# thebarnable/sparch

Measured on AMD Instinct MI355X. Metric: train-step timesteps*samples/sec (fwd+bwd+Adam), RadLIF 3x1024 SSC shape, higher is better.
Workload: dtype f32; 1 GPU; RadLIF [1024, 1024, 35] batchnorm pdrop=0.1, B=256/GPU T=250 C=700 Bernoulli(0.05) spikes (BASELINE.json configs[2]); global_batch=256, seq_len=250, parallelism=dp1, sync_bn=False, launch=eager (auto: host enqueue 2.58 ms of a 6.64 ms step during warm-up), operands=fp32 through exact bf16 splits

## Files before the change

sparch_amd/csrc/gemm_spike.hip:

```cpp
#include <cstdlib>
#include <type_traits>
#include "common.h"

namespace {

typedef unsigned u32x4 __attribute__((ext_vector_type(4)));
typedef unsigned u32x2 __attribute__((ext_vector_type(2)));
typedef short s16x4 __attribute__((ext_vector_type(4)));
typedef __bf16 bf16x8 __attribute__((ext_vector_type(8)));
typedef __attribute__((address_space(3))) s16x4 lds_s16x4;

constexpr int BK = 32;
constexpr int TAIL2 = 2;
constexpr int KC_ROW = 40;
template <int ROWS> constexpr int km_row() { return ROWS + 32; }
template <bool KM, int ROWS> constexpr int plane_elems() { return KM ? BK * km_row<ROWS>() : ROWS * KC_ROW; }

enum Epi { EPI_NONE = 0, EPI_BIAS = 1, EPI_STATS = 2 };

#ifdef SPARCH_REC_PROF
__device__ unsigned long long g_gemm_prof[8 + 8 * 2];
#define GP_DECL                                                                                  \
    unsigned long long gp_t = 0, gp_acc[5] = {0, 0, 0, 0, 0}, gp_c0, gp_r0;                      \
    asm volatile("s_memtime %0\n\ts_memrealtime %1\n\ts_waitcnt lgkmcnt(0)" : "=s"(gp_c0), "=s"(gp_r0)::"memory");
#define GP_STAMP(i)                                                                              \
    do {                                                                                         \
        unsigned long long now_;                                                                 \
        __builtin_amdgcn_sched_barrier(0);                                                       \
        asm volatile("s_memtime %0\n\ts_waitcnt lgkmcnt(0)" : "=s"(now_)::"memory");           \
        __builtin_amdgcn_sched_barrier(0);                                                       \
        if ((i) >= 0) gp_acc[(i) < 0 ? 0 : (i)] += now_ - gp_t;                                  \
        gp_t = now_;                                                                             \
    } while (0)
#define GP_FLUSH()                                                                               \
    if ((threadIdx.x & 63) == 0 && blockIdx.x == 7) {                                            \
        atomicAdd(&g_gemm_prof[8 + 2 * (threadIdx.x >> 6)], gp_acc[3]);                          \
        atomicAdd(&g_gemm_prof[9 + 2 * (threadIdx.x >> 6)], gp_acc[4]);                          \
    }                                                                                            \
    if (threadIdx.x == 0 && blockIdx.x == 7) {                                                   \
        unsigned long long c1_, r1_;                                                             \
        asm volatile("s_memtime %0\n\ts_memrealtime %1\n\ts_waitcnt lgkmcnt(0)" : "=s"(c1_), "=s"(r1_)::"memory"); \
        for (int i_ = 0; i_ < 5; ++i_) atomicAdd(&g_gemm_prof[i_], gp_acc[i_]);                  \
        atomicAdd(&g_gemm_prof[5], c1_ - gp_c0);                                                 \
        atomicAdd(&g_gemm_prof[6], r1_ - gp_r0);                                                 \
    }
#else
#define GP_DECL
#define GP_STAMP(i)
#define GP_FLUSH()
#endif

struct SArgs {
    const float* A; const float* B; float* C;
    const float* bias; float* colstat;
    int M, N, K, lda, ldb, ldc;
    int k_per_split; size_t c_split_stride;
    int a_vec, b_vec;
    float scale;
    const unsigned* gate; unsigned gate_want;
    int e_exact;
    const unsigned short* Bp; size_t bp_stride;
    const unsigned short* Ap; size_t ap_stride;
    int n_splits;
};

__device__ __forceinline__ unsigned short bf16_bits(float x) {
    return __builtin_bit_cast(unsigned short, (__bf16)x);
}
__device__ __forceinline__ void split3(float x, unsigned short& hi, unsigned short& mid, unsigned short& lo) {
    const __bf16 h = (__bf16)x;
    const float r1 = x - (float)h;
    const __bf16 m = (__bf16)r1;
    const float r2 = r1 - (float)m;
    hi = __builtin_bit_cast(unsigned short, h);
    mid = __builtin_bit_cast(unsigned short, m);
    lo = bf16_bits(r2);
}

template <bool KM, int ROWS>
__device__ __forceinline__ bool tile_is_full(int row0, int rows, int k0, int kend, int vec) {
    return vec && row0 + ROWS <= rows && k0 + BK <= kend;
}
__device__ __forceinline__ f32x4 ld16(const void* q) { return *reinterpret_cast<const f32x4*>(q); }
template <int PPR>
__device__ __forceinline__ void rm_piece(int f, int& row, int& kp) { row = f / PPR; kp = f % PPR; }
template <bool KM, int ROWS, int NT>
__device__ __forceinline__ void load_piece(f32x4& out, int p, bool fast, const float* __restrict__ P, int ld,
                                           int row0, int rows, int k0, int kend, int vec, int tid) {
    constexpr int RQ = ROWS / 4;
    const int f = tid + NT * p;
    int row, k;
    if constexpr (!KM) { int r_, kp_; rm_piece<8>(f, r_, kp_); row = row0 + r_; k = k0 + (kp_ << 2); }
    else               { k = k0 + f / RQ; row = row0 + ((f % RQ) << 2); }
    if (fast) {
        if constexpr (!KM) out = ld16(P + (size_t)row * ld + k);
        else               out = ld16(P + (size_t)k * ld + row);
        return;
    }
    f32x4 v = {0.f, 0.f, 0.f, 0.f};
    if constexpr (!KM) {
        if (row < rows) {
            const float* q = P + (size_t)row * ld + k;
            if (vec && k + 3 < kend) v = *reinterpret_cast<const f32x4*>(q);
            else {
                if (k + 0 < kend) v.x = q[0];
                if (k + 1 < kend) v.y = q[1];
                if (k + 2 < kend) v.z = q[2];
                if (k + 3 < kend) v.w = q[3];
            }
        }
    } else {
        if (k < kend) {
            const float* q = P + (size_t)k * ld + row;
            if (vec && row + 3 < rows) v = *reinterpret_cast<const f32x4*>(q);
            else {
                if (row + 0 < rows) v.x = q[0];
// ... 76 lines not shown
            const float r0 = r[2 * pr] - __uint_as_float(x0 & 0xFFFF0000u);
            const float r1 = r[2 * pr + 1] - __uint_as_float(x1 & 0xFFFF0000u);
            const unsigned y0 = __float_as_uint(r0), y1 = __float_as_uint(r1);
            const float q0 = r0 - __uint_as_float(y0 & 0xFFFF0000u);
            const float q1 = r1 - __uint_as_float(y1 & 0xFFFF0000u);
            w1[pr] = __builtin_amdgcn_perm(x1, x0, 0x07060302u);
            w2[pr] = __builtin_amdgcn_perm(y1, y0, 0x07060302u);
            w3[pr] = __builtin_amdgcn_perm(__float_as_uint(q1), __float_as_uint(q0), 0x07060302u);
        }
        *reinterpret_cast<u32x2*>(S + off) = w1;
        *reinterpret_cast<u32x2*>(S + PLANE + off) = w2;
        *reinterpret_cast<u32x2*>(S + 2 * PLANE + off) = w3;
    } else {
        unsigned short h[4], m[4], l[4];
#pragma unroll
        for (int e = 0; e < 4; ++e) split3(r[e], h[e], m[e], l[e]);
        *reinterpret_cast<u32x2*>(S + off) = u32x2{(unsigned)h[0] | ((unsigned)h[1] << 16), (unsigned)h[2] | ((unsigned)h[3] << 16)};
        *reinterpret_cast<u32x2*>(S + PLANE + off) = u32x2{(unsigned)m[0] | ((unsigned)m[1] << 16), (unsigned)m[2] | ((unsigned)m[3] << 16)};
        *reinterpret_cast<u32x2*>(S + 2 * PLANE + off) = u32x2{(unsigned)l[0] | ((unsigned)l[1] << 16), (unsigned)l[2] | ((unsigned)l[3] << 16)};
    }
}
template <bool KM, int ROWS, int NT>
__device__ __forceinline__ void store_piece_rne1(const f32x4& r, int p, unsigned short* __restrict__ S, int tid) {
    constexpr int RQ = ROWS / 4;
    typedef __bf16 bf16x2 __attribute__((ext_vector_type(2)));
    const int f = tid + NT * p;
    int off;
    if constexpr (!KM) { int r_, kp_; rm_piece<8>(f, r_, kp_); off = r_ * KC_ROW + (kp_ << 2); }
    else               off = (f / RQ) * km_row<ROWS>() + ((f % RQ) << 2);
    u32x2 w;
    w.x = __builtin_bit_cast(unsigned, bf16x2{(__bf16)r.x, (__bf16)r.y});
    w.y = __builtin_bit_cast(unsigned, bf16x2{(__bf16)r.z, (__bf16)r.w});
    *reinterpret_cast<u32x2*>(S + off) = w;
}
template <bool KM, int ROWS>
__device__ __forceinline__ u32x4 frag_read(const unsigned short* __restrict__ S, int idx_base, int lane, int ks) {
    constexpr int KM_ROW = km_row<ROWS>();
    if constexpr (!KM) {
        const int r = lane & 31, h = lane >> 5;
        return *reinterpret_cast<const u32x4*>(S + (idx_base + r) * KC_ROW + 16 * ks + 8 * h);
    } else {
        const int g = lane >> 4, i = lane & 15, q = i >> 2, p4 = i & 3;
        const int col = idx_base + 16 * (g & 1) + 4 * p4;
        const int k0 = 16 * ks + 8 * (g >> 1);
        const unsigned short* a0 = S + (k0 + q) * KM_ROW + col;
        const u32x2 lo = __builtin_bit_cast(u32x2, __builtin_amdgcn_ds_read_tr16_b64_v4i16((lds_s16x4*)(a0)));
        const u32x2 hi = __builtin_bit_cast(u32x2, __builtin_amdgcn_ds_read_tr16_b64_v4i16((lds_s16x4*)(a0 + 4 * KM_ROW)));
        return u32x4{lo.x, lo.y, hi.x, hi.y};
    }
}

__device__ __forceinline__ f32x16 mfma_bf16(u32x4 a, u32x4 b, f32x16 c) {
    return __builtin_amdgcn_mfma_f32_32x32x16_bf16(__builtin_bit_cast(bf16x8, a), __builtin_bit_cast(bf16x8, b), c, 0, 0, 0);
}

template <int MODE, bool FAST, bool BIG = false> struct Shape {
    static constexpr int WM = FAST ? (MODE == 1 ? 4 : 2) : 2;
    static constexpr int WN = FAST ? (MODE == 1 ? 2 : 4) : 2;
    static constexpr int WI = FAST ? (MODE == 0 ? 4 : (MODE == 1 ? (BIG ? 2 : 1) : (BIG ? 4 : 2))) : 2;
    static constexpr int WJ = FAST ? (MODE == 1 ? 4 : (BIG ? 2 : 1)) : 2;
    static constexpr int BM = 32 * WI * WM, BN = 32 * WJ * WN;
    static constexpr int NT = 64 * WM * WN;
    static constexpr int OCC = FAST ? 1 : (MODE == 2 ? 2 : 3);
};

template <bool A_KM, bool B_KM, int MODE, bool FAST, int NP>
constexpr bool big_tile() { return FAST && ((A_KM && B_KM && MODE != 2) || NP == 1); }

extern __shared__ __attribute__((aligned(16))) unsigned short dyn_lds[];

template <bool A_KM, bool B_KM, int MODE, bool FAST, int NP = 3>
constexpr int stage_elems() {
    using S = Shape<MODE, FAST, big_tile<A_KM, B_KM, MODE, FAST, NP>()>;
    return (MODE == 0 ? 1 : NP) * plane_elems<A_KM, S::BM>() + (MODE == 1 ? 1 : NP) * plane_elems<B_KM, S::BN>();
}

template <bool A_KM, bool B_KM, int MODE, int EPI, bool FAST, bool S16, bool BPRE = false, int NP = 3, bool APRE = false>
__global__ __launch_bounds__((Shape<MODE, FAST>::NT), (Shape<MODE, FAST>::OCC)) void gemm_spike_kernel(SArgs g) {
    static_assert(!S16 || MODE != 2, "a bf16 plane is a spike operand");
    static_assert(!BPRE || (FAST && MODE != 1), "pre-split B: pipelined kernel, B is the dense operand");
    static_assert(!APRE || (FAST && MODE != 0 && NP == 3), "pre-split A: pipelined exact kernel, A is the dense operand");
    static_assert(NP == 3 || (NP == 1 && !BPRE), "dense operands: three exact planes or one rounded plane");
    constexpr bool BIGT = big_tile<A_KM, B_KM, MODE, FAST, NP>();
    using S = Shape<MODE, FAST, BIGT>;
    constexpr bool SPIKE_A = MODE == 0;
    constexpr bool SPIKE_B = MODE == 1;
    constexpr int WI = S::WI, WJ = S::WJ, WN = S::WN, BM = S::BM, BN = S::BN, NT = S::NT;
    constexpr int A_PLANES = SPIKE_A ? 1 : NP;
    [[maybe_unused]] constexpr int B_PLANES = SPIKE_B ? 1 : NP;
    constexpr int PLANE_A = plane_elems<A_KM, BM>(), PLANE_B = plane_elems<B_KM, BN>();
    constexpr int STAGE = stage_elems<A_KM, B_KM, MODE, FAST, NP>();
    unsigned short* const lds = dyn_lds;

    if (g.gate != nullptr && *g.gate != g.gate_want) return;
    const int tid = threadIdx.x;
    const int lane = tid & 63, wave = tid >> 6;
    const int li = lane & 31, h = lane >> 5;
    const int wm = wave / WN, wn = wave % WN;
    const int tiles_n = (g.N + BN - 1) / BN;
    const int tiles_all = tiles_n * ((g.M + BM - 1) / BM);
    const int total = tiles_all * g.n_splits;
    const int xcd = blockIdx.x & 7, idx = blockIdx.x >> 3;
    const int wgs_here = (gridDim.x >> 3) + (xcd < (int)(gridDim.x & 7) ? 1 : 0);
    const int lin_end = (xcd + 1) * (total >> 3) + min(xcd + 1, total & 7);
    constexpr bool WALKS = FAST && !BIGT;
    int lin = xcd * (total >> 3) + min(xcd, total & 7) + idx;
// ... 227 lines not shown
    for (int j = 0; j < WJ; ++j) {
        csum[j] = 0.f; csq[j] = 0.f;
        const int col = n0 + (wn * WJ + j) * 32 + li;
        float bj = 0.f;
        if constexpr (EPI & EPI_BIAS) bj = (g.bias != nullptr && (FAST || col < g.N)) ? g.bias[col] : 0.f;
#pragma unroll
        for (int i = 0; i < WI; ++i) {
#pragma unroll
            for (int r = 0; r < 16; ++r) {
                const int row = m0 + (wm * WI + i) * 32 + (r & 3) + 8 * (r >> 2) + 4 * h;
                float v = acc[i][j][r] * g.scale;
                if constexpr (EPI & EPI_BIAS) v = v + bj;
                if (FAST || (row < g.M && col < g.N)) {
                    Cz[(size_t)row * g.ldc + col] = v;
                    if constexpr (EPI & EPI_STATS) { csum[j] += v; csq[j] += v * v; }
                }
            }
        }
    }
    if constexpr (EPI & EPI_STATS) {
        float* red = reinterpret_cast<float*>(lds);
#pragma unroll
        for (int j = 0; j < WJ; ++j) {
            csum[j] += __shfl_xor(csum[j], 32);
            csq[j] += __shfl_xor(csq[j], 32);
        }
        if (h == 0) {
#pragma unroll
            for (int j = 0; j < WJ; ++j) {
                const int c = (wn * WJ + j) * 32 + li;
                red[(0 * 2 + wm) * BN + c] = csum[j];
                red[(1 * 2 + wm) * BN + c] = csq[j];
            }
        }
        __syncthreads();
        if (tid < BN && n0 + tid < g.N && g.colstat != nullptr) {
            const int blocks = (g.M + 127) / 128;
            if constexpr (WI == 2) {
                g.colstat[(size_t)tile_m * g.N + n0 + tid] = red[0 * BN + tid] + red[1 * BN + tid];
                g.colstat[(size_t)(blocks + tile_m) * g.N + n0 + tid] = red[2 * BN + tid] + red[3 * BN + tid];
            } else {
                static_assert(WI == 2 || WI == 4, "colstat blocks are 128 rows");
#pragma unroll
                for (int w = 0; w < 2; ++w) {
                    const int blk = 2 * tile_m + w;
                    if (blk < blocks) {
                        g.colstat[(size_t)blk * g.N + n0 + tid] = red[(0 * 2 + w) * BN + tid];
                        g.colstat[(size_t)(blocks + blk) * g.N + n0 + tid] = red[(1 * 2 + w) * BN + tid];
                    }
                }
            }
        }
    }
    __syncthreads();
    } while (WALKS && (lin += wgs_here) < lin_end);
}

__global__ void splitk_reduce_kernel2(const float* __restrict__ ws, float* __restrict__ C, int M, int N, int ldc,
                                      int splits, int zero_diag, int accumulate, int ld_ws = 0) {
    const size_t i = (size_t)blockIdx.x * blockDim.x + threadIdx.x;
    const size_t total = (size_t)M * N;
    if (i >= total) return;
    const int m = (int)(i / N), n = (int)(i % N);
    const size_t lw = ld_ws ? (size_t)ld_ws : (size_t)N, slab = (size_t)M * lw, at = (size_t)m * lw + n;
    float s = 0.f;
    for (int z = 0; z < splits; ++z) s += ws[(size_t)z * slab + at];
    if (zero_diag && m == n) s = 0.f;
    float* c = C + (size_t)m * ldc + n;
    *c = accumulate ? (*c + s) : s;
}

int target_wgs(int occ) {
    static const int env = [] { const char* e = getenv("SPARCH_GEMM_TARGET_WGS"); return e ? atoi(e) : 0; }();
    if (env > 0) return env;
    static const int cus = [] {
        int dev = 0, n = 256;
        if (hipGetDevice(&dev) == hipSuccess) (void)hipDeviceGetAttribute(&n, hipDeviceAttributeMultiprocessorCount, dev);
        return n;
    }();
    return occ * cus;
}
template <int MODE>
int choose_splits(int M, int N, int K) {
    if (sparch_operand_bf16()) {
        using SB = Shape<MODE, true, true>;
        const int tiles_b = cdiv(M, SB::BM) * cdiv(N, SB::BN);
        int sb = target_wgs(1) / tiles_b;
        if (sb > cdiv(K, BK) / 8) sb = cdiv(K, BK) / 8;
        return sb < 1 ? 1 : sb;
    }
    using S = Shape<MODE, true, MODE != 2>;
    const int tiles = cdiv(M, S::BM) * cdiv(N, S::BN);
    const int kt = cdiv(K, BK);
    int s = target_wgs(1) / tiles;
    if (s > kt / 8) s = kt / 8;
    return s < 1 ? 1 : s;
}

template <bool A_KM, bool B_KM, int MODE, int EPI, bool S16, int NP = 3>
bool fast_ok(const SArgs& g) {
    using S = Shape<MODE, true, big_tile<A_KM, B_KM, MODE, true, NP>()>;
    constexpr int BM = S::BM, BN = S::BN;
    constexpr int QA = (S16 && MODE == 0) ? 8 : 4, QB = (S16 && MODE == 1) ? 8 : 4;
    return g.a_vec && g.b_vec && g.M >= BM && g.N >= BN && (!A_KM || g.M % QA == 0) && (!B_KM || g.N % QB == 0) &&
           (!(EPI & EPI_STATS) || g.M % BM == 0) && g.k_per_split % BK == 0 &&
           g.k_per_split >= 8 * BK;
}

template <bool A_KM, bool B_KM, int MODE, int EPI, bool FAST, bool S16, bool BPRE = false, int NP = 3, bool APRE = false>
int launch_variant(SArgs& g, int splits, hipStream_t st) {
    constexpr bool BIGT = big_tile<A_KM, B_KM, MODE, FAST, NP>();
    using S = Shape<MODE, FAST, BIGT>;
    const int work = cdiv(g.M, S::BM) * cdiv(g.N, S::BN) * splits;
    g.n_splits = splits;
    static const bool persistent = [] { const char* e = getenv("SPARCH_GEMM_PERSISTENT"); return !e || atoi(e) != 0; }();
    const int cus = target_wgs(1);
    const int wgs = (FAST && !BIGT && persistent && work > cus) ? cus : work;
    constexpr size_t lds_bytes = (size_t)(FAST ? 2 : 1) * stage_elems<A_KM, B_KM, MODE, FAST, NP>() * sizeof(unsigned short);
    auto kernel = gemm_spike_kernel<A_KM, B_KM, MODE, EPI, FAST, S16, BPRE, NP, APRE>;
    static const hipError_t attr = hipFuncSetAttribute(reinterpret_cast<const void*>(kernel),
                                                       hipFuncAttributeMaxDynamicSharedMemorySize, (int)lds_bytes);
    if (attr != hipSuccess) { sparch_note_hip_error((int)attr); return SPARCH_ELAUNCH; }
    hipLaunchKernelGGL(kernel, dim3(wgs, 1, 1), dim3(Shape<MODE, FAST>::NT), lds_bytes, st, g);
    SPARCH_CHECK_LAUNCH();
    return SPARCH_OK;
}

template <bool A_KM, bool B_KM, int MODE, int EPI, bool S16 = false>
int launch(SArgs& g, int splits, hipStream_t st) {
    if (sparch_operand_bf16()) {
        if (fast_ok<A_KM, B_KM, MODE, EPI, S16, 1>(g))
            return launch_variant<A_KM, B_KM, MODE, EPI, true, S16, false, 1>(g, splits, st);
        return launch_variant<A_KM, B_KM, MODE, EPI, false, S16, false, 1>(g, splits, st);
    }
    if (fast_ok<A_KM, B_KM, MODE, EPI, S16>(g)) return launch_variant<A_KM, B_KM, MODE, EPI, true, S16>(g, splits, st);
    return launch_variant<A_KM, B_KM, MODE, EPI, false, S16>(g, splits, st);
}
template <bool A_KM, bool B_KM, int MODE, int EPI, bool S16 = false>
int launch_wp(SArgs& g, int splits, hipStream_t st) {
    const bool planes_ok = g.Bp != nullptr && aligned16(g.Bp) && g.ldb % 8 == 0 && (g.bp_stride % 8) == 0 &&
                           g.k_per_split % BK == 0 && g.K % BK == 0 && (!B_KM || g.N % 8 == 0);
    if (planes_ok && !sparch_operand_bf16() && fast_ok<A_KM, B_KM, MODE, EPI, S16>(g))
        return launch_variant<A_KM, B_KM, MODE, EPI, true, S16, true>(g, splits, st);
    return launch<A_KM, B_KM, MODE, EPI, S16>(g, splits, st);
}

template <bool A_KM, bool B_KM, int MODE, int EPI, bool S16, bool BPRE>
int launch_ap(SArgs& g, int splits, hipStream_t st) {
    const bool a_ok = g.Ap != nullptr && aligned16(g.Ap) && g.lda % 8 == 0 && (g.ap_stride % 8) == 0 &&
// ... 29 lines not shown
}

}

extern "C" int sparch_split3(size_t n, const float* x, uint16_t* planes, void* stream) {
    SPARCH_ENTER();
    if (n == 0 || n % 8 != 0 || !x || !planes) return SPARCH_EINVAL;
    if (!aligned16(x) || !aligned16(planes)) return SPARCH_EALIGN;
    const size_t n4 = n / 4;
    hipLaunchKernelGGL(split3_kernel, dim3((unsigned)((n4 + 255) / 256)), dim3(256), 0, (hipStream_t)stream, n4,
                       reinterpret_cast<const u32x4*>(x), reinterpret_cast<u32x2*>(planes),
                       reinterpret_cast<u32x2*>(planes + n), reinterpret_cast<u32x2*>(planes + 2 * n));
    SPARCH_CHECK_LAUNCH();
    return SPARCH_OK;
}

extern "C" int sparch_gemm_spike_nt(int M, int N, int K, const float* A_spk, int lda, float scale, const float* B,
                                    int ldb, float* C, int ldc, const float* bias, float* colstat_ws,
                                    void* stream, int precision) {
    SPARCH_ENTER();
    PrecisionScope prec_scope_(precision);
    if (!prec_scope_.ok) return SPARCH_EINVAL;
    if (M <= 0 || N <= 0 || K <= 0 || !A_spk || !B || !C || lda < K || ldb < K || ldc < N) return SPARCH_EINVAL;
    SArgs g{};
    g.A = A_spk; g.B = B; g.C = C; g.bias = bias; g.colstat = colstat_ws;
    g.M = M; g.N = N; g.K = K; g.lda = lda; g.ldb = ldb; g.ldc = ldc;
    g.k_per_split = cdiv(K, BK) * BK; g.c_split_stride = 0; g.scale = scale;
    g.a_vec = aligned16(A_spk) && (lda % 4 == 0);
    g.b_vec = aligned16(B) && (ldb % 4 == 0);
    hipStream_t st = (hipStream_t)stream;
    if (colstat_ws) return launch<false, false, 0, EPI_BIAS | EPI_STATS>(g, 1, st);
    if (bias) return launch<false, false, 0, EPI_BIAS>(g, 1, st);
    return launch<false, false, 0, EPI_NONE>(g, 1, st);
}

extern "C" int sparch_gemm_spike_tn(int M, int N, int K, const float* A, int lda, const float* B, int ldb,
                                    int spike_side, float scale, float* C, int ldc, int zero_diag,
                                    int accumulate, void* ws, size_t ws_bytes, void* stream, int precision) {
    SPARCH_ENTER();
    PrecisionScope prec_scope_(precision);
    if (!prec_scope_.ok) return SPARCH_EINVAL;
    if (M <= 0 || N <= 0 || K <= 0 || !A || !B || !C || lda < M || ldb < N || ldc < N) return SPARCH_EINVAL;
    if (spike_side != 0 && spike_side != 1) return SPARCH_EINVAL;
    hipStream_t st = (hipStream_t)stream;
    const int splits = spike_side == 0 ? choose_splits<0>(M, N, K) : choose_splits<1>(M, N, K);
    const size_t need = (size_t)splits * M * N * sizeof(float);
    if (!ws || ws_bytes < need) return SPARCH_EWORKSPACE;
    SArgs g{};
    g.A = A; g.B = B; g.M = M; g.N = N; g.K = K; g.lda = lda; g.ldb = ldb; g.scale = scale;
    g.a_vec = aligned16(A) && (lda % 4 == 0);
    g.b_vec = aligned16(B) && (ldb % 4 == 0);
    g.C = (float*)ws; g.ldc = N; g.c_split_stride = (size_t)M * N;
    g.k_per_split = cdiv(cdiv(K, splits), BK) * BK;
    int rc = spike_side == 0 ? launch<true, true, 0, EPI_NONE>(g, splits, st)
                             : launch<true, true, 1, EPI_NONE>(g, splits, st);
    if (rc != SPARCH_OK) return rc;
    const size_t total = (size_t)M * N;
    hipLaunchKernelGGL(splitk_reduce_kernel2, dim3((unsigned)((total + 255) / 256)), dim3(256), 0, st,
                       (const float*)ws, C, M, N, ldc, splits, zero_diag, accumulate);
    SPARCH_CHECK_LAUNCH();
    return SPARCH_OK;
}

extern "C" int sparch_gemm_spike16_nt(int M, int N, int K, const uint16_t* A_spk16, int lda, float scale,
                                      const float* B, int ldb, float* C, int ldc, const float* bias,
                                      float* colstat_ws, void* stream, int precision) {
    SPARCH_ENTER();
    PrecisionScope prec_scope_(precision);
    if (!prec_scope_.ok) return SPARCH_EINVAL;
    if (M <= 0 || N <= 0 || K <= 0 || !A_spk16 || !B || !C || lda < K || ldb < K || ldc < N) return SPARCH_EINVAL;
    SArgs g{};
    g.A = reinterpret_cast<const float*>(A_spk16); g.B = B; g.C = C; g.bias = bias; g.colstat = colstat_ws;
    g.M = M; g.N = N; g.K = K; g.lda = lda; g.ldb = ldb; g.ldc = ldc;
    g.k_per_split = cdiv(K, BK) * BK; g.c_split_stride = 0; g.scale = scale;
    g.a_vec = aligned16(A_spk16) && (lda % 8 == 0);
    g.b_vec = aligned16(B) && (ldb % 4 == 0);
    hipStream_t st = (hipStream_t)stream;
    if (colstat_ws) return launch<false, false, 0, EPI_BIAS | EPI_STATS, true>(g, 1, st);
    if (bias) return launch<false, false, 0, EPI_BIAS, true>(g, 1, st);
    return launch<false, false, 0, EPI_NONE, true>(g, 1, st);
}

extern "C" int sparch_gemm_spike16_nt_wp(int M, int N, int K, const uint16_t* A_spk16, int lda, float scale,
                                         const float* B, const uint16_t* B_planes, int ldb, float* C, int ldc,
                                         const float* bias, float* colstat_ws, void* stream, int precision) {
    SPARCH_ENTER();
    PrecisionScope prec_scope_(precision);
    if (!prec_scope_.ok) return SPARCH_EINVAL;
    if (M <= 0 || N <= 0 || K <= 0 || !A_spk16 || !B || !C || lda < K || ldb < K || ldc < N) return SPARCH_EINVAL;
    SArgs g{};
    g.A = reinterpret_cast<const float*>(A_spk16); g.B = B; g.C = C; g.bias = bias; g.colstat = colstat_ws;
    g.Bp = B_planes; g.bp_stride = (size_t)N * ldb;
    g.M = M; g.N = N; g.K = K; g.lda = lda; g.ldb = ldb; g.ldc = ldc;
    g.k_per_split = cdiv(K, BK) * BK; g.c_split_stride = 0; g.scale = scale;
    g.a_vec = aligned16(A_spk16) && (lda % 8 == 0);
    g.b_vec = aligned16(B) && (ldb % 4 == 0);
    hipStream_t st = (hipStream_t)stream;
    if (colstat_ws) return launch_wp<false, false, 0, EPI_BIAS | EPI_STATS, true>(g, 1, st);
    if (bias) return launch_wp<false, false, 0, EPI_BIAS, true>(g, 1, st);
    return launch_wp<false, false, 0, EPI_NONE, true>(g, 1, st);
}

extern "C" int sparch_gemm6_nn_wp(int M, int N, int K, const float* A, int lda, const float* B,
                                  const uint16_t* B_planes, int ldb, float* C, int ldc, void* stream, int precision) {
    SPARCH_ENTER();
    PrecisionScope prec_scope_(precision);
    if (!prec_scope_.ok) return SPARCH_EINVAL;
    if (M <= 0 || N <= 0 || K <= 0 || !A || !B || !C || lda < K || ldb < N || ldc < N) return SPARCH_EINVAL;
    SArgs g{};
    g.A = A; g.B = B; g.C = C; g.Bp = B_planes; g.bp_stride = (size_t)K * ldb;
    g.M = M; g.N = N; g.K = K; g.lda = lda; g.ldb = ldb; g.ldc = ldc;
    g.k_per_split = cdiv(K, BK) * BK; g.c_split_stride = 0; g.scale = 1.0f;
    g.a_vec = aligned16(A) && (lda % 4 == 0);
    g.b_vec = aligned16(B) && (ldb % 4 == 0);
    return launch_wp<false, true, 2, EPI_NONE>(g, 1, (hipStream_t)stream);
}

extern "C" int sparch_gemm_spike16_tn(int M, int N, int K, const void* A, int lda, const void* B, int ldb,
                                      int spike_side, float scale, float* C, int ldc, int zero_diag,
                                      int accumulate, void* ws, size_t ws_bytes, void* stream, int precision) {
    SPARCH_ENTER();
    PrecisionScope prec_scope_(precision);
    if (!prec_scope_.ok) return SPARCH_EINVAL;
    if (M <= 0 || N <= 0 || K <= 0 || !A || !B || !C || lda < M || ldb < N || ldc < N) return SPARCH_EINVAL;
    if (spike_side != 0 && spike_side != 1) return SPARCH_EINVAL;
    hipStream_t st = (hipStream_t)stream;
    const int splits = spike_side == 0 ? choose_splits<0>(M, N, K) : choose_splits<1>(M, N, K);
    const size_t need = (size_t)splits * M * N * sizeof(float);
    if (!ws || ws_bytes < need) return SPARCH_EWORKSPACE;
    SArgs g{};
    g.A = static_cast<const float*>(A); g.B = static_cast<const float*>(B);
    g.M = M; g.N = N; g.K = K; g.lda = lda; g.ldb = ldb; g.scale = scale;
    g.a_vec = aligned16(A) && (lda % (spike_side == 0 ? 8 : 4) == 0);
    g.b_vec = aligned16(B) && (ldb % (spike_side == 1 ? 8 : 4) == 0);
    g.C = (float*)ws; g.ldc = N; g.c_split_stride = (size_t)M * N;
    g.k_per_split = cdiv(cdiv(K, splits), BK) * BK;
    int rc = spike_side == 0 ? launch<true, true, 0, EPI_NONE, true>(g, splits, st)
                             : launch<true, true, 1, EPI_NONE, true>(g, splits, st);
    if (rc != SPARCH_OK) return rc;
    const size_t total = (size_t)M * N;
    hipLaunchKernelGGL(splitk_reduce_kernel2, dim3((unsigned)((total + 255) / 256)), dim3(256), 0, st,
                       (const float*)ws, C, M, N, ldc, splits, zero_diag, accumulate);
    SPARCH_CHECK_LAUNCH();
    return SPARCH_OK;
}

extern "C" int sparch_gemm6_nn_pp(int M, int N, int K, const float* A, const uint16_t* A_planes, int lda, const float* B,
                                  const uint16_t* B_planes, int ldb, float* C, int ldc, void* stream, int precision) {
    SPARCH_ENTER();
    PrecisionScope prec_scope_(precision);
    if (!prec_scope_.ok) return SPARCH_EINVAL;
    if (M <= 0 || N <= 0 || K <= 0 || (!A && !A_planes) || !B || !C || lda < K || ldb < N || ldc < N) return SPARCH_EINVAL;
    SArgs g{};
    g.A = A; g.B = B; g.C = C; g.Bp = B_planes; g.bp_stride = (size_t)K * ldb;
    g.Ap = A_planes; g.ap_stride = (size_t)M * lda;
    g.M = M; g.N = N; g.K = K; g.lda = lda; g.ldb = ldb; g.ldc = ldc;
    g.k_per_split = cdiv(K, BK) * BK; g.c_split_stride = 0; g.scale = 1.0f;
    g.a_vec = (A ? aligned16(A) : true) && (lda % 4 == 0);
    g.b_vec = aligned16(B) && (ldb % 4 == 0);
    return launch_ap<false, true, 2, EPI_NONE, false, true>(g, 1, (hipStream_t)stream);
}

extern "C" int sparch_gemm_spike16_tn_ap(int M, int N, int K, const float* A, const uint16_t* A_planes, int lda,
                                         const uint16_t* B16, int ldb, float scale, float* C, int ldc, int zero_diag,
                                         int accumulate, void* ws, size_t ws_bytes, void* stream, int precision) {
    SPARCH_ENTER();
    PrecisionScope prec_scope_(precision);
    if (!prec_scope_.ok) return SPARCH_EINVAL;
    if (M <= 0 || N <= 0 || K <= 0 || (!A && !A_planes) || !B16 || !C || lda < M || ldb < N || ldc < N) return SPARCH_EINVAL;
    hipStream_t st = (hipStream_t)stream;
    const int splits = choose_splits<1>(M, N, K);
    const size_t need = (size_t)splits * M * N * sizeof(float);
    if (!ws || ws_bytes < need) return SPARCH_EWORKSPACE;
    SArgs g{};
    g.A = A; g.B = reinterpret_cast<const float*>(B16);
    g.Ap = A_planes; g.ap_stride = (size_t)K * lda;
    g.M = M; g.N = N; g.K = K; g.lda = lda; g.ldb = ldb; g.scale = scale;
    g.a_vec = (A ? aligned16(A) : true) && (lda % 4 == 0);
    g.b_vec = aligned16(B16) && (ldb % 8 == 0);
    g.C = (float*)ws; g.ldc = N; g.c_split_stride = (size_t)M * N;
    g.k_per_split = cdiv(cdiv(K, splits), BK) * BK;
    int rc = launch_ap<true, true, 1, EPI_NONE, true, false>(g, splits, st);
    if (rc != SPARCH_OK) return rc;
    const size_t total = (size_t)M * N;
    hipLaunchKernelGGL(splitk_reduce_kernel2, dim3((unsigned)((total + 255) / 256)), dim3(256), 0, st,
                       (const float*)ws, C, M, N, ldc, splits, zero_diag, accumulate);
    SPARCH_CHECK_LAUNCH();
    return SPARCH_OK;
}

extern "C" int sparch_gemm6_nt(int M, int N, int K, const float* A, int lda, const float* B, int ldb, float* C,
                               int ldc, const float* bias, float* colstat_ws, void* stream, int precision) {
    SPARCH_ENTER();
    PrecisionScope prec_scope_(precision);
    if (!prec_scope_.ok) return SPARCH_EINVAL;
    if (M <= 0 || N <= 0 || K <= 0 || !A || !B || !C || lda < K || ldb < K || ldc < N) return SPARCH_EINVAL;
    SArgs g{};
    g.A = A; g.B = B; g.C = C; g.bias = bias; g.colstat = colstat_ws;
    g.M = M; g.N = N; g.K = K; g.lda = lda; g.ldb = ldb; g.ldc = ldc;
    g.k_per_split = cdiv(K, BK) * BK; g.c_split_stride = 0; g.scale = 1.0f;
    g.a_vec = aligned16(A) && (lda % 4 == 0);
    g.b_vec = aligned16(B) && (ldb % 4 == 0);
    hipStream_t st = (hipStream_t)stream;
    if (colstat_ws) return launch<false, false, 2, EPI_BIAS | EPI_STATS>(g, 1, st);
    if (bias) return launch<false, false, 2, EPI_BIAS>(g, 1, st);
    return launch<false, false, 2, EPI_NONE>(g, 1, st);
}

extern "C" int sparch_gemm6_nn(int M, int N, int K, const float* A, int lda, const float* B, int ldb, float* C,
                               int ldc, void* stream, int precision) {
    SPARCH_ENTER();
    PrecisionScope prec_scope_(precision);
    if (!prec_scope_.ok) return SPARCH_EINVAL;
    if (M <= 0 || N <= 0 || K <= 0 || !A || !B || !C || lda < K || ldb < N || ldc < N) return SPARCH_EINVAL;
    SArgs g{};
    g.A = A; g.B = B; g.C = C;
    g.M = M; g.N = N; g.K = K; g.lda = lda; g.ldb = ldb; g.ldc = ldc;
    g.k_per_split = cdiv(K, BK) * BK; g.c_split_stride = 0; g.scale = 1.0f;
    g.a_vec = aligned16(A) && (lda % 4 == 0);
    g.b_vec = aligned16(B) && (ldb % 4 == 0);
    return launch<false, true, 2, EPI_NONE>(g, 1, (hipStream_t)stream);
}

namespace {
int small_splits(int M, int N, int K) {
    using S = Shape<2, true>;
    const int tiles = cdiv(M, S::BM) * cdiv(N, S::BN);
    const int kt = cdiv(K, BK);
    int s = target_wgs(1) / tiles;
    if (s > kt / 8) s = kt / 8;
    return s < 1 ? 1 : s;
}
template <bool B_KM>
int gemm6_splitk(int M, int N, int K, const float* A, int lda, const float* B, int ldb, float* C, int ldc, void* ws,
                 size_t ws_bytes, hipStream_t st) {
    const int splits = small_splits(M, N, K);
    SArgs g{};
    g.A = A; g.B = B; g.M = M; g.N = N; g.K = K; g.lda = lda; g.ldb = ldb; g.scale = 1.0f;
    g.a_vec = aligned16(A) && (lda % 4 == 0);
    g.b_vec = aligned16(B) && (ldb % 4 == 0);
    if (splits == 1) {
        g.C = C; g.ldc = ldc; g.k_per_split = cdiv(K, BK) * BK; g.c_split_stride = 0;
        return launch<false, B_KM, 2, EPI_NONE>(g, 1, st);
    }
    if (!ws || ws_bytes < (size_t)splits * M * N * sizeof(float)) return SPARCH_EWORKSPACE;
    g.C = (float*)ws; g.ldc = N; g.c_split_stride = (size_t)M * N;
    g.k_per_split = cdiv(cdiv(K, splits), BK) * BK;
    int rc = launch<false, B_KM, 2, EPI_NONE>(g, splits, st);
    if (rc != SPARCH_OK) return rc;
    const size_t total = (size_t)M * N;
    hipLaunchKernelGGL(splitk_reduce_kernel2, dim3((unsigned)((total + 255) / 256)), dim3(256), 0, st,
                       (const float*)ws, C, M, N, ldc, splits, 0, 0);
    SPARCH_CHECK_LAUNCH();
    return SPARCH_OK;
}
}

extern "C" size_t sparch_gemm6_splitk_workspace_bytes(int M, int N, int K, int precision) {
    PrecisionScope prec_scope_(precision);
    if (!prec_scope_.ok) return 0;
    if (M <= 0 || N <= 0 || K <= 0) return 0;
    const int s = small_splits(M, N, K);
    return s > 1 ? (size_t)s * M * N * sizeof(float) : 0;
}
extern "C" int sparch_gemm6_nt_splitk(int M, int N, int K, const float* A, int lda, const float* B, int ldb,
                                      float* C, int ldc, void* ws, size_t ws_bytes, void* stream, int precision) {
    SPARCH_ENTER();
    PrecisionScope prec_scope_(precision);
    if (!prec_scope_.ok) return SPARCH_EINVAL;
    if (M <= 0 || N <= 0 || K <= 0 || !A || !B || !C || lda < K || ldb < K || ldc < N) return SPARCH_EINVAL;
    return gemm6_splitk<false>(M, N, K, A, lda, B, ldb, C, ldc, ws, ws_bytes, (hipStream_t)stream);
}
extern "C" int sparch_gemm6_nn_splitk(int M, int N, int K, const float* A, int lda, const float* B, int ldb,
                                      float* C, int ldc, void* ws, size_t ws_bytes, void* stream, int precision) {
    SPARCH_ENTER();
    PrecisionScope prec_scope_(precision);
    if (!prec_scope_.ok) return SPARCH_EINVAL;
    if (M <= 0 || N <= 0 || K <= 0 || !A || !B || !C || lda < K || ldb < N || ldc < N) return SPARCH_EINVAL;
    return gemm6_splitk<true>(M, N, K, A, lda, B, ldb, C, ldc, ws, ws_bytes, (hipStream_t)stream);
}

extern "C" int sparch_gemm6_tn(int M, int N, int K, const float* A, int lda, const float* B, int ldb, float* C,
                               int ldc, int zero_diag, int accumulate, void* ws, size_t ws_bytes, void* stream, int precision) {
    SPARCH_ENTER();
    PrecisionScope prec_scope_(precision);
    if (!prec_scope_.ok) return SPARCH_EINVAL;
    if (M <= 0 || N <= 0 || K <= 0 || !A || !B || !C || lda < M || ldb < N || ldc < N) return SPARCH_EINVAL;
    hipStream_t st = (hipStream_t)stream;
    const int splits = choose_splits<2>(M, N, K);
    const size_t need = (size_t)splits * M * N * sizeof(float);
    if (!ws || ws_bytes < need) return SPARCH_EWORKSPACE;
    SArgs g{};
    g.A = A; g.B = B; g.M = M; g.N = N; g.K = K; g.lda = lda; g.ldb = ldb; g.scale = 1.0f;
    g.a_vec = aligned16(A) && (lda % 4 == 0);
    g.b_vec = aligned16(B) && (ldb % 4 == 0);
    g.C = (float*)ws; g.ldc = N; g.c_split_stride = (size_t)M * N;
    g.k_per_split = cdiv(cdiv(K, splits), BK) * BK;
    int rc = launch<true, true, 2, EPI_NONE>(g, splits, st);
    if (rc != SPARCH_OK) return rc;
    const size_t total = (size_t)M * N;
    hipLaunchKernelGGL(splitk_reduce_kernel2, dim3((unsigned)((total + 255) / 256)), dim3(256), 0, st,
                       (const float*)ws, C, M, N, ldc, splits, zero_diag, accumulate);
    SPARCH_CHECK_LAUNCH();
    return SPARCH_OK;
}

__global__ void flag_bf16_exact_kernel(size_t n4, const u32x4* __restrict__ x, unsigned* __restrict__ flag) {
    const size_t i = (size_t)blockIdx.x * blockDim.x + threadIdx.x;
    unsigned bad = 0;
    for (size_t j = i; j < n4; j += (size_t)gridDim.x * blockDim.x) {
        const u32x4 v = x[j];
        bad |= (v.x | v.y | v.z | v.w) & 0xFFFFu;
    }
    if (__any(bad != 0) && (threadIdx.x & 63) == 0) atomicAnd(flag, 0u);
}
__global__ void flag_set_kernel(unsigned* flag, unsigned v) { *flag = v; }

extern "C" int sparch_flag_bf16_exact(size_t n, const float* x, uint32_t* flag, void* stream) {
    SPARCH_ENTER();
    if (n == 0 || !x || !flag) return SPARCH_EINVAL;
    hipStream_t st = (hipStream_t)stream;
    const bool vec = aligned16(x) && (n % 4 == 0);
    hipLaunchKernelGGL(flag_set_kernel, dim3(1), dim3(1), 0, st, flag, vec ? 1u : 0u);
    SPARCH_CHECK_LAUNCH();
    if (vec) {
        hipLaunchKernelGGL(flag_bf16_exact_kernel, dim3(2048), dim3(256), 0, st, n / 4,
                           reinterpret_cast<const u32x4*>(x), flag);
        SPARCH_CHECK_LAUNCH();
    }
    return SPARCH_OK;
}

extern "C" int sparch_gemm_auto_nt(int M, int N, int K, const float* A, int lda, const float* B, int ldb,
                                   float* C, int ldc, const float* bias, float* colstat_ws,
                                   const uint32_t* a_exact_flag, void* stream, int precision) {
    SPARCH_ENTER();
    PrecisionScope prec_scope_(precision);
    if (!prec_scope_.ok) return SPARCH_EINVAL;
    if (M <= 0 || N <= 0 || K <= 0 || !A || !B || !C || lda < K || ldb < K || ldc < N || !a_exact_flag)
        return SPARCH_EINVAL;
    SArgs g{};
    g.A = A; g.B = B; g.C = C; g.bias = bias; g.colstat = colstat_ws;
    g.M = M; g.N = N; g.K = K; g.lda = lda; g.ldb = ldb; g.ldc = ldc;
    g.k_per_split = cdiv(K, BK) * BK; g.c_split_stride = 0; g.scale = 1.0f;
    g.a_vec = aligned16(A) && (lda % 4 == 0);
    g.b_vec = aligned16(B) && (ldb % 4 == 0);
    g.gate = a_exact_flag; g.e_exact = 1;
    hipStream_t st = (hipStream_t)stream;
    int rc;
    g.gate_want = 1;
    if (colstat_ws) rc = launch<false, false, 0, EPI_BIAS | EPI_STATS>(g, 1, st);
    else rc = launch<false, false, 0, EPI_BIAS>(g, 1, st);
    if (rc != SPARCH_OK) return rc;
    g.gate_want = 0;
    if (colstat_ws) return launch<false, false, 2, EPI_BIAS | EPI_STATS>(g, 1, st);
    return launch<false, false, 2, EPI_BIAS>(g, 1, st);
}

extern "C" int sparch_gemm_auto_tn(int M, int N, int K, const float* A, int lda, const float* B, int ldb,
                                   float* C, int ldc, int zero_diag, int accumulate,
                                   const uint32_t* b_exact_flag, void* ws, size_t ws_bytes, void* stream, int precision) {
    SPARCH_ENTER();
    PrecisionScope prec_scope_(precision);
    if (!prec_scope_.ok) return SPARCH_EINVAL;
    if (M <= 0 || N <= 0 || K <= 0 || !A || !B || !C || lda < M || ldb < N || ldc < N || !b_exact_flag)
        return SPARCH_EINVAL;
    hipStream_t st = (hipStream_t)stream;
    const int splits = choose_splits<1>(M, N, K);
    const size_t need = (size_t)splits * M * N * sizeof(float);
    if (!ws || ws_bytes < need) return SPARCH_EWORKSPACE;
    SArgs g{};
    g.A = A; g.B = B; g.M = M; g.N = N; g.K = K; g.lda = lda; g.ldb = ldb; g.scale = 1.0f;
    g.a_vec = aligned16(A) && (lda % 4 == 0);
    g.b_vec = aligned16(B) && (ldb % 4 == 0);
    g.C = (float*)ws; g.ldc = N; g.c_split_stride = (size_t)M * N;
    g.k_per_split = cdiv(cdiv(K, splits), BK) * BK;
    g.gate = b_exact_flag; g.e_exact = 1;
    g.gate_want = 1;
    int rc = launch<true, true, 1, EPI_NONE>(g, splits, st);
    if (rc != SPARCH_OK) return rc;
    g.gate_want = 0;
    rc = launch<true, true, 2, EPI_NONE>(g, splits, st);
    if (rc != SPARCH_OK) return rc;
    const size_t total = (size_t)M * N;
    hipLaunchKernelGGL(splitk_reduce_kernel2, dim3((unsigned)((total + 255) / 256)), dim3(256), 0, st,
                       (const float*)ws, C, M, N, ldc, splits, zero_diag, accumulate);
    SPARCH_CHECK_LAUNCH();
    return SPARCH_OK;
}

__global__ void plane_flag_kernel(int M, int K, int ldx, int ldp, const float* __restrict__ x,
                                  unsigned short* __restrict__ plane, unsigned* __restrict__ flag) {
    const int q = ldp / 4;
    const size_t total = (size_t)M * q;
    unsigned bad = 0;
    for (size_t i = (size_t)blockIdx.x * blockDim.x + threadIdx.x; i < total; i += (size_t)gridDim.x * blockDim.x) {
        const size_t m = i / q;
        const int k = (int)(i - m * q) * 4;
        unsigned w[4];
#pragma unroll
        for (int e = 0; e < 4; ++e) w[e] = (k + e < K) ? __float_as_uint(x[m * ldx + k + e]) : 0u;
        bad |= (w[0] | w[1] | w[2] | w[3]) & 0xFFFFu;
        u32x2 o;
        o.x = (w[0] >> 16) | (w[1] & 0xFFFF0000u);
        o.y = (w[2] >> 16) | (w[3] & 0xFFFF0000u);
        *reinterpret_cast<u32x2*>(plane + m * ldp + k) = o;
    }
    if (__any(bad != 0) && (threadIdx.x & 63) == 0) atomicAnd(flag, 0u);
}

extern "C" int sparch_plane_bf16_exact(int M, int K, const float* x, int ldx, uint16_t* plane, int ldp,
                                       uint32_t* flag, void* stream) {
    SPARCH_ENTER();
    if (M <= 0 || K <= 0 || !x || !plane || !flag || ldx < K || ldp < K || ldp % 8 != 0) return SPARCH_EINVAL;
    if (!aligned16(plane)) return SPARCH_EALIGN;
    hipStream_t st = (hipStream_t)stream;
    hipLaunchKernelGGL(flag_set_kernel, dim3(1), dim3(1), 0, st, flag, 1u);
    SPARCH_CHECK_LAUNCH();
    hipLaunchKernelGGL(plane_flag_kernel, dim3(2048), dim3(256), 0, st, M, K, ldx, ldp, x, plane, flag);
    SPARCH_CHECK_LAUNCH();
    return SPARCH_OK;
}

extern "C" int sparch_gemm_auto16_nt(int M, int N, int K, const float* A, int lda, const uint16_t* A16, int lda16,
                                     const float* B, int ldb, float* C, int ldc, const float* bias,
                                     float* colstat_ws, const uint32_t* a_exact_flag, void* stream, int precision) {
    SPARCH_ENTER();
    PrecisionScope prec_scope_(precision);
    if (!prec_scope_.ok) return SPARCH_EINVAL;
    if (M <= 0 || N <= 0 || K <= 0 || !A || !A16 || !B || !C || lda < K || lda16 < K || ldb < K || ldc < N ||
        !a_exact_flag)
        return SPARCH_EINVAL;
    SArgs g{};
    g.B = B; g.C = C; g.bias = bias; g.colstat = colstat_ws;
    g.M = M; g.N = N; g.K = K; g.ldb = ldb; g.ldc = ldc;
    g.k_per_split = cdiv(K, BK) * BK; g.c_split_stride = 0; g.scale = 1.0f;
    g.b_vec = aligned16(B) && (ldb % 4 == 0);
    g.gate = a_exact_flag; g.e_exact = 1;
    hipStream_t st = (hipStream_t)stream;
    g.A = reinterpret_cast<const float*>(A16); g.lda = lda16;
    g.a_vec = aligned16(A16) && (lda16 % 8 == 0);
    g.gate_want = 1;
    int rc = colstat_ws ? launch<false, false, 0, EPI_BIAS | EPI_STATS, true>(g, 1, st)
                        : launch<false, false, 0, EPI_BIAS, true>(g, 1, st);
    if (rc != SPARCH_OK) return rc;
    g.A = A; g.lda = lda; g.a_vec = aligned16(A) && (lda % 4 == 0);
    g.gate_want = 0;
    if (colstat_ws) return launch<false, false, 2, EPI_BIAS | EPI_STATS>(g, 1, st);
    return launch<false, false, 2, EPI_BIAS>(g, 1, st);
}

extern "C" int sparch_gemm_auto16_tn(int M, int N, int K, const float* A, int lda, const float* B, int ldb,
                                     const uint16_t* B16, int ldb16, float* C, int ldc, int zero_diag,
                                     int accumulate, const uint32_t* b_exact_flag, void* ws, size_t ws_bytes,
                                     void* stream, int precision) {
    SPARCH_ENTER();
    PrecisionScope prec_scope_(precision);
    if (!prec_scope_.ok) return SPARCH_EINVAL;
    if (M <= 0 || N <= 0 || K <= 0 || !A || !B || !B16 || !C || lda < M || ldb < N || ldb16 < N || ldc < N ||
        !b_exact_flag)
        return SPARCH_EINVAL;
    hipStream_t st = (hipStream_t)stream;
    const int N8 = (N + 7) & ~7;
    if (N8 > ldb16) return SPARCH_EINVAL;
    const int splits = choose_splits<1>(M, N8, K);
    const size_t need = (size_t)splits * M * N8 * sizeof(float);
    if (!ws || ws_bytes < need) return SPARCH_EWORKSPACE;
    SArgs g{};
    g.A = A; g.M = M; g.N = N8; g.K = K; g.lda = lda; g.scale = 1.0f;
    g.a_vec = aligned16(A) && (lda % 4 == 0);
    g.C = (float*)ws; g.ldc = N8; g.c_split_stride = (size_t)M * N8;
    g.k_per_split = cdiv(cdiv(K, splits), BK) * BK;
    g.gate = b_exact_flag; g.e_exact = 1;
    g.B = reinterpret_cast<const float*>(B16); g.ldb = ldb16;
    g.b_vec = aligned16(B16) && (ldb16 % 8 == 0);
    g.gate_want = 1;
    int rc = launch<true, true, 1, EPI_NONE, true>(g, splits, st);
    if (rc != SPARCH_OK) return rc;
    g.N = N;
    g.B = B; g.ldb = ldb; g.b_vec = aligned16(B) && (ldb % 4 == 0);
    g.gate_want = 0;
    rc = launch<true, true, 2, EPI_NONE>(g, splits, st);
    if (rc != SPARCH_OK) return rc;
    const size_t total = (size_t)M * N;
    hipLaunchKernelGGL(splitk_reduce_kernel2, dim3((unsigned)((total + 255) / 256)), dim3(256), 0, st,
                       (const float*)ws, C, M, N, ldc, splits, zero_diag, accumulate, N8);
    SPARCH_CHECK_LAUNCH();
    return SPARCH_OK;
}

#ifdef SPARCH_REC_PROF
extern "C" int sparch_gemm_prof_read(unsigned long long* host_out, int reset) {
    static unsigned long long zero[8 + 8 * 2];
    if (hipMemcpyFromSymbol(host_out, HIP_SYMBOL(g_gemm_prof), sizeof(zero)) != hipSuccess) return -1;
    if (reset && hipMemcpyToSymbol(HIP_SYMBOL(g_gemm_prof), zero, sizeof(zero)) != hipSuccess) return -1;
    return 0;
}
#endif

extern "C" size_t sparch_gemm_spike_tn_workspace_bytes(int M, int N, int K, int precision) {
    PrecisionScope prec_scope_(precision);
    if (!prec_scope_.ok) return 0;
    if (M <= 0 || N <= 0 || K <= 0) return 0;
    const int s0 = choose_splits<0>(M, N, K), s1 = choose_splits<1>(M, N, K), s2 = choose_splits<2>(M, N, K);
    const int smax = s0 > s1 ? (s0 > s2 ? s0 : s2) : (s1 > s2 ? s1 : s2);
    return (size_t)smax * M * N * sizeof(float);
}
```

Before: 10.47 million timesteps*samples/s.

## Fuse split-K reduction into GEMM via last-arriving workgroup per tile

```diff
diff --git a/sparch_amd/csrc/gemm_spike.hip b/sparch_amd/csrc/gemm_spike.hip
--- a/sparch_amd/csrc/gemm_spike.hip
+++ b/sparch_amd/csrc/gemm_spike.hip
@@ -1,5 +1,8 @@
 #include <cstdlib>
+#include <map>
+#include <mutex>
 #include <type_traits>
+#include <utility>
 #include "common.h"
 
 namespace {
@@ -62,6 +65,9 @@
     const unsigned short* Bp; size_t bp_stride;
     const unsigned short* Ap; size_t ap_stride;
     int n_splits;
+    float* Cf; int ldcf, n_out, zero_diag, accumulate;
+    int fin_vec;
+    unsigned* tile_cnt;
 };
 
 __device__ __forceinline__ unsigned short bf16_bits(float x) {
@@ -244,6 +250,67 @@
 
 __device__ __forceinline__ f32x16 mfma_bf16(u32x4 a, u32x4 b, f32x16 c) {
     return __builtin_amdgcn_mfma_f32_32x32x16_bf16(__builtin_bit_cast(bf16x8, a), __builtin_bit_cast(bf16x8, b), c, 0, 0, 0);
+}
+
+template <typename V, int NT>
+__device__ __forceinline__ void sum_slabs(const SArgs& g, int m0, int n0, int bm, int bn, int tid) {
+    constexpr int VW = sizeof(V) / sizeof(float);
+    const int rows = min(bm, g.M - m0), cols = min(bn, g.n_out - n0) / VW;
+    const int total = rows * cols;
+    const size_t stride = g.c_split_stride;
+#pragma unroll 1
+    for (int e0 = tid; e0 < total; e0 += 4 * NT) {
+        const float* p[4];
+        V s[4];
+#pragma unroll
+        for (int k = 0; k < 4; ++k) {
+            const int e = min(e0 + k * NT, total - 1);
+            const int r = e / cols, c = (e - r * cols) * VW;
+            p[k] = g.C + (size_t)(m0 + r) * g.ldc + n0 + c;
+            s[k] = V{};
+        }
+        int z = 0;
+#pragma unroll 1
+        for (; z + 4 <= g.n_splits; z += 4) {
+            V t[4][4];
+#pragma unroll
+            for (int u = 0; u < 4; ++u)
+#pragma unroll
+                for (int k = 0; k < 4; ++k) t[u][k] = *reinterpret_cast<const V*>(p[k] + u * stride);
+#pragma unroll
+            for (int u = 0; u < 4; ++u)
+#pragma unroll
+                for (int k = 0; k < 4; ++k) s[k] += t[u][k];
+#pragma unroll
+            for (int k = 0; k < 4; ++k) p[k] += 4 * stride;
+        }
+#pragma unroll 1
+        for (; z < g.n_splits; ++z) {
+            V t[4];
+#pragma unroll
+            for (int k = 0; k < 4; ++k) t[k] = *reinterpret_cast<const V*>(p[k]);
+#pragma unroll
+            for (int k = 0; k < 4; ++k) { s[k] += t[k]; p[k] += stride; }
+        }
+#pragma unroll
+        for (int k = 0; k < 4; ++k) {
+            const int e = e0 + k * NT;
+            if (e < total) {
+                const int r = e / cols, c = (e - r * cols) * VW;
+                const int row = m0 + r, col = n0 + c;
+                V v = s[k];
+                if (g.zero_diag) {
+                    if constexpr (VW == 1) { if (row == col) v = 0.f; }
+                    else {
+#pragma unroll
+                        for (int q = 0; q < VW; ++q) if (row == col + q) v[q] = 0.f;
+                    }
+                }
+                V* c_out = reinterpret_cast<V*>(g.Cf + (size_t)row * g.ldcf + col);
+                if (g.accumulate) *c_out = *c_out + v; else *c_out = v;
+            }
+        }
+    }
 }
 
 template <int MODE, bool FAST, bool BIG = false> struct Shape {
@@ -577,6 +644,33 @@
             }
         }
     }
+    if constexpr (EPI == EPI_NONE) {
+        if (g.Cf != nullptr) {
+            unsigned* const last_flag = reinterpret_cast<unsigned*>(lds);
+            asm volatile("s_waitcnt vmcnt(0)" ::: "memory");
+            __syncthreads();
+            if (tid == 0) {
+                bool last = true;
+                if (g.n_splits > 1) {
+                    __builtin_amdgcn_fence(__ATOMIC_RELEASE, "agent");
+                    asm volatile("s_waitcnt vmcnt(0)" ::: "memory");
+                    const unsigned old = __hip_atomic_fetch_add(g.tile_cnt + tile, 1u, __ATOMIC_RELAXED, __HIP_MEMORY_SCOPE_AGENT);
+                    last = old == (unsigned)(g.n_splits - 1);
+                    if (last) {
+                        __hip_atomic_store(g.tile_cnt + tile, 0u, __ATOMIC_RELAXED, __HIP_MEMORY_SCOPE_AGENT);
+                        __builtin_amdgcn_fence(__ATOMIC_ACQUIRE, "agent");
+                        asm volatile("s_waitcnt vmcnt(0)" ::: "memory");
+                    }
+                }
+                *last_flag = last ? 1u : 0u;
+            }
+            __syncthreads();
+            if (*last_flag != 0u) {
+                if (g.fin_vec) sum_slabs<f32x4, NT>(g, tile_m * BM, tile_n * BN, BM, BN, tid);
+                else sum_slabs<float, NT>(g, tile_m * BM, tile_n * BN, BM, BN, tid);
+            }
+        }
+    }
     __syncthreads();
     } while (WALKS && (lin += wgs_here) < lin_end);
 }
@@ -620,6 +714,63 @@
     int s = target_wgs(1) / tiles;
     if (s > kt / 8) s = kt / 8;
     return s < 1 ? 1 : s;
+}
+
+bool fused_reduce_enabled() {
+    static const bool on = [] { const char* e = getenv("SPARCH_GEMM_FUSED_REDUCE"); return !e || atoi(e) != 0; }();
+    return on;
+}
+constexpr size_t FUSED_MAX_TILE_BYTES = (size_t)1 << 20;
+constexpr int MAX_TILE = 256, MIN_TILE = 128;
+constexpr int CNT_PER_BLOCK = 1024, CNT_BLOCKS = 512;
+struct CounterPool {
+    unsigned* base = nullptr;
+    std::map<std::pair<hipStream_t, unsigned long long>, int> block_of;
+};
+unsigned* tile_counters(hipStream_t st) {
+    static std::mutex mu;
+    static std::map<int, CounterPool> pools;
+    hipStreamCaptureStatus cap = hipStreamCaptureStatusNone;
+    unsigned long long cap_id = 0;
+    int dev = 0;
+    if (hipStreamGetCaptureInfo(st, &cap, &cap_id) != hipSuccess || hipGetDevice(&dev) != hipSuccess) {
+        (void)hipGetLastError();
+        return nullptr;
+    }
+    const bool capturing = cap != hipStreamCaptureStatusNone;
+    std::lock_guard<std::mutex> lock(mu);
+    CounterPool& pool = pools[dev];
+    if (pool.base == nullptr) {
+        if (capturing) return nullptr;
+        const size_t bytes = (size_t)CNT_BLOCKS * CNT_PER_BLOCK * sizeof(unsigned);
+        unsigned* p = nullptr;
+        if (hipMalloc(reinterpret_cast<void**>(&p), bytes) != hipSuccess || hipMemset(p, 0, bytes) != hipSuccess) {
+            (void)hipGetLastError();
+            if (p) (void)hipFree(p);
+            return nullptr;
+        }
+        pool.base = p;
+    }
+    const auto key = std::make_pair(st, capturing ? cap_id : 0ull);
+    auto it = pool.block_of.find(key);
+    if (it == pool.block_of.end()) {
+        if ((int)pool.block_of.size() >= CNT_BLOCKS) return nullptr;
+        it = pool.block_of.emplace(key, (int)pool.block_of.size()).first;
+    }
+    return pool.base + (size_t)it->second * CNT_PER_BLOCK;
+}
+bool fuse_reduce(SArgs& g, int splits, hipStream_t st, float* C, int ldc, int n_out, int zero_diag, int accumulate) {
+    if (!fused_reduce_enabled()) return false;
+    if (splits > 1) {
+        const size_t tile_bytes = (size_t)splits * (g.M < MAX_TILE ? g.M : MAX_TILE) * (g.N < MAX_TILE ? g.N : MAX_TILE) * sizeof(float);
+        if (tile_bytes > FUSED_MAX_TILE_BYTES) return false;
+        if ((long long)cdiv(g.M, MIN_TILE) * cdiv(g.N, MIN_TILE) > CNT_PER_BLOCK) return false;
+        g.tile_cnt = tile_counters(st);
+        if (g.tile_cnt == nullptr) return false;
+    }
+    g.Cf = C; g.ldcf = ldc; g.n_out = n_out; g.zero_diag = zero_diag; g.accumulate = accumulate;
+    g.fin_vec = aligned16(g.C) && g.ldc % 4 == 0 && g.c_split_stride % 4 == 0 && aligned16(C) && ldc % 4 == 0 && n_out % 4 == 0;
+    return true;
 }
 
 template <bool A_KM, bool B_KM, int MODE, int EPI, bool S16, int NP = 3>
@@ -755,9 +906,11 @@
     g.b_vec = aligned16(B) && (ldb % 4 == 0);
     g.C = (float*)ws; g.ldc = N; g.c_split_stride = (size_t)M * N;
     g.k_per_split = cdiv(cdiv(K, splits), BK) * BK;
+    const bool fused = fuse_reduce(g, splits, st, C, ldc, N, zero_diag, accumulate);
     int rc = spike_side == 0 ? launch<true, true, 0, EPI_NONE>(g, splits, st)
                              : launch<true, true, 1, EPI_NONE>(g, splits, st);
     if (rc != SPARCH_OK) return rc;
+    if (fused) return SPARCH_OK;
     const size_t total = (size_t)M * N;
     hipLaunchKernelGGL(splitk_reduce_kernel2, dim3((unsigned)((total + 255) / 256)), dim3(256), 0, st,
                        (const float*)ws, C, M, N, ldc, splits, zero_diag, accumulate);
@@ -838,9 +991,11 @@
     g.b_vec = aligned16(B) && (ldb % (spike_side == 1 ? 8 : 4) == 0);
     g.C = (float*)ws; g.ldc = N; g.c_split_stride = (size_t)M * N;
     g.k_per_split = cdiv(cdiv(K, splits), BK) * BK;
+    const bool fused = fuse_reduce(g, splits, st, C, ldc, N, zero_diag, accumulate);
     int rc = spike_side == 0 ? launch<true, true, 0, EPI_NONE, true>(g, splits, st)
                              : launch<true, true, 1, EPI_NONE, true>(g, splits, st);
     if (rc != SPARCH_OK) return rc;
+    if (fused) return SPARCH_OK;
     const size_t total = (size_t)M * N;
     hipLaunchKernelGGL(splitk_reduce_kernel2, dim3((unsigned)((total + 255) / 256)), dim3(256), 0, st,
                        (const float*)ws, C, M, N, ldc, splits, zero_diag, accumulate);
@@ -883,8 +1038,10 @@
     g.b_vec = aligned16(B16) && (ldb % 8 == 0);
     g.C = (float*)ws; g.ldc = N; g.c_split_stride = (size_t)M * N;
     g.k_per_split = cdiv(cdiv(K, splits), BK) * BK;
+    const bool fused = fuse_reduce(g, splits, st, C, ldc, N, zero_diag, accumulate);
     int rc = launch_ap<true, true, 1, EPI_NONE, true, false>(g, splits, st);
     if (rc != SPARCH_OK) return rc;
+    if (fused) return SPARCH_OK;
     const size_t total = (size_t)M * N;
     hipLaunchKernelGGL(splitk_reduce_kernel2, dim3((unsigned)((total + 255) / 256)), dim3(256), 0, st,
                        (const float*)ws, C, M, N, ldc, splits, zero_diag, accumulate);
@@ -949,8 +1106,10 @@
     if (!ws || ws_bytes < (size_t)splits * M * N * sizeof(float)) return SPARCH_EWORKSPACE;
     g.C = (float*)ws; g.ldc = N; g.c_split_stride = (size_t)M * N;
     g.k_per_split = cdiv(cdiv(K, splits), BK) * BK;
+    const bool fused = fuse_reduce(g, splits, st, C, ldc, N, 0, 0);
     int rc = launch<false, B_KM, 2, EPI_NONE>(g, splits, st);
     if (rc != SPARCH_OK) return rc;
+    if (fused) return SPARCH_OK;
     const size_t total = (size_t)M * N;
     hipLaunchKernelGGL(splitk_reduce_kernel2, dim3((unsigned)((total + 255) / 256)), dim3(256), 0, st,
                        (const float*)ws, C, M, N, ldc, splits, 0, 0);
@@ -999,8 +1158,10 @@
     g.b_vec = aligned16(B) && (ldb % 4 == 0);
     g.C = (float*)ws; g.ldc = N; g.c_split_stride = (size_t)M * N;
     g.k_per_split = cdiv(cdiv(K, splits), BK) * BK;
+    const bool fused = fuse_reduce(g, splits, st, C, ldc, N, zero_diag, accumulate);
     int rc = launch<true, true, 2, EPI_NONE>(g, splits, st);
     if (rc != SPARCH_OK) return rc;
+    if (fused) return SPARCH_OK;
     const size_t total = (size_t)M * N;
     hipLaunchKernelGGL(splitk_reduce_kernel2, dim3((unsigned)((total + 255) / 256)), dim3(256), 0, st,
                        (const float*)ws, C, M, N, ldc, splits, zero_diag, accumulate);
@@ -1079,12 +1240,14 @@
     g.C = (float*)ws; g.ldc = N; g.c_split_stride = (size_t)M * N;
     g.k_per_split = cdiv(cdiv(K, splits), BK) * BK;
     g.gate = b_exact_flag; g.e_exact = 1;
+    const bool fused = fuse_reduce(g, splits, st, C, ldc, N, zero_diag, accumulate);
     g.gate_want = 1;
     int rc = launch<true, true, 1, EPI_NONE>(g, splits, st);
     if (rc != SPARCH_OK) return rc;
     g.gate_want = 0;
     rc = launch<true, true, 2, EPI_NONE>(g, splits, st);
     if (rc != SPARCH_OK) return rc;
+    if (fused) return SPARCH_OK;
     const size_t total = (size_t)M * N;
     hipLaunchKernelGGL(splitk_reduce_kernel2, dim3((unsigned)((total + 255) / 256)), dim3(256), 0, st,
                        (const float*)ws, C, M, N, ldc, splits, zero_diag, accumulate);
@@ -1175,6 +1338,7 @@
     g.C = (float*)ws; g.ldc = N8; g.c_split_stride = (size_t)M * N8;
     g.k_per_split = cdiv(cdiv(K, splits), BK) * BK;
     g.gate = b_exact_flag; g.e_exact = 1;
+    const bool fused = fuse_reduce(g, splits, st, C, ldc, N, zero_diag, accumulate);
     g.B = reinterpret_cast<const float*>(B16); g.ldb = ldb16;
     g.b_vec = aligned16(B16) && (ldb16 % 8 == 0);
     g.gate_want = 1;
@@ -1185,6 +1349,7 @@
     g.gate_want = 0;
     rc = launch<true, true, 2, EPI_NONE>(g, splits, st);
     if (rc != SPARCH_OK) return rc;
+    if (fused) return SPARCH_OK;
     const size_t total = (size_t)M * N;
     hipLaunchKernelGGL(splitk_reduce_kernel2, dim3((unsigned)((total + 255) / 256)), dim3(256), 0, st,
                        (const float*)ws, C, M, N, ldc, splits, zero_diag, accumulate, N8);
```

Result: slower. 10.31 million timesteps*samples/s (-1.5%).
